# shamim-hussain/egt

Hardware: AMD Instinct MI355X
Metric: graphs/sec EGT fwd+bwd, ZINC-500K padded N=64 (higher is better)
Workload: dtype f32; 1 GPU; zinc500k_n64: attention-block stack (h,e,mask)->(h',e') x Ly, fwd+bwd + param grads; scope=stack, graphs_per_gpu=128, global_batch=128, N=64, Dh=64, De=64, H=8, d=8, Ly=10, parallelism=dp1, grad_allreduce_bytes=740480, backend=none (single process), flat_grad_adopted=True, flat_grad_bound=True, collective_in_graph=False

## Files before the change

egt_amd/_lib.py:

```python
from __future__ import annotations

import ctypes as C
import os

_HERE = os.path.dirname(os.path.abspath(__file__))
LIB_PATH = os.environ.get("EGT_AMD_LIB") or os.path.join(_HERE, "lib", "libegt_amd.so")

ABI_VERSION = 4
EGT_OK = 0
EGT_E_NULL, EGT_E_SHAPE, EGT_E_DTYPE, EGT_E_FLAGS, EGT_E_HIP, EGT_E_WORKSPACE, EGT_E_RCCL = -1, -2, -3, -4, -5, -6, -7
EGT_F32 = 0
EGT_BF16 = 1
F_EDGE_INPUT, F_GATE_INPUT, F_ATTN_MASK, F_SCALE_DEGREE = 0x001, 0x002, 0x004, 0x008
F_SCALER_LINEAR, F_TRAINING, F_CLIP = 0x010, 0x020, 0x040
ATTN_WS_SHARED = 0x1
EP_LAYERNORM, EP_GATES = 0x1, 0x2
ACT_NONE, ACT_LRELU, ACT_RELU, ACT_ELU = 0, 1, 2, 3
BF_GATE, BF_ATTN_MASK, BF_TRAINING, BF_CLIP, BF_NO_EDGE_LN, BF_SEED_DEVICE = 0x1, 0x2, 0x4, 0x8, 0x10, 0x20
BF_STATIC_EDGE = 0x40


class AttnDesc(C.Structure):
    _fields_ = [("B", C.c_int32), ("N", C.c_int32), ("H", C.c_int32), ("d", C.c_int32),
                ("dtype", C.c_int32), ("flags", C.c_uint32),
# ... 151 lines not shown
    "egt_dp_init": (C.c_int, [_VP, C.c_int32, C.c_int32]),
    "egt_dp_allreduce": (C.c_int, [_VP, C.c_size_t, C.c_int32, _VP]),
    "egt_dp_world": (C.c_int, []),
    "egt_dp_rank": (C.c_int, []),
    "egt_dp_finalize": (C.c_int, []),
    "egt_prof_enable": (C.c_int, [C.c_int]),
    "egt_prof_filter": (C.c_int, [C.c_char_p]),
    "egt_prof_stride": (C.c_int, [C.c_int]),
    "egt_prof_read": (C.c_int, [C.c_char_p, C.POINTER(C.c_int64), C.POINTER(C.c_double)]),
    "egt_prof_names": (C.c_int, [C.c_char_p, C.c_size_t]),
    "egt_prof_collect_graph": (C.c_int, [C.c_int]),
    "egt_prof_forget_graphs": (C.c_int, []),
    "egt_block_supported": (C.c_int, [C.POINTER(BlockDesc)]),
    "egt_block_bwd_kernel": (C.c_char_p, [C.POINTER(BlockDesc)]),
    "egt_block_launch_form": (C.c_char_p, [C.POINTER(BlockDesc)]),
    "egt_block_saved_bytes": (C.c_size_t, [C.POINTER(BlockDesc)]),
    "egt_block_workspace_bytes": (C.c_size_t, [C.POINTER(BlockDesc)]),
    "egt_block_fwd": (C.c_int, [C.POINTER(BlockDesc), C.POINTER(BlockParams)] + [_VP] * 10),
    "egt_block_bwd": (C.c_int, [C.POINTER(BlockDesc), C.POINTER(BlockParams)] + [_VP] * 10
                      + [C.POINTER(BlockParams)] + [_VP] * 2),
    "egt_stack_saved_bytes": (C.c_size_t, [C.POINTER(BlockDesc), C.c_int32]),
    "egt_stack_workspace_bytes": (C.c_size_t, [C.POINTER(BlockDesc), C.c_int32]),
    "egt_stack_fwd": (C.c_int, [C.POINTER(BlockDesc), C.c_int32, C.POINTER(BlockParams)] + [_VP] * 9),
    "egt_stack_bwd": (C.c_int, [C.POINTER(BlockDesc), C.c_int32, C.POINTER(BlockParams)] + [_VP] * 9
                      + [C.POINTER(BlockParams)] + [_VP] * 2),
    "egt_pair_supported": (C.c_int, [C.POINTER(BlockDesc)]),
    "egt_pair_workspace_bytes": (C.c_size_t, [C.POINTER(BlockDesc)]),
    "egt_pair_fwd": (C.c_int, [C.POINTER(BlockDesc), C.POINTER(BlockParams)] + [_VP] * 8),
    "egt_pair_bwd": (C.c_int, [C.POINTER(BlockDesc), C.POINTER(BlockParams)] + [_VP] * 9
                     + [C.POINTER(BlockParams)] + [_VP] * 2),
# ... 45 lines not shown
```

egt_amd/csrc/egt_block.h:

```cpp
#pragma once
#include "egt_common.h"

typedef float v4f __attribute__((ext_vector_type(4)));
#define MFMA(a, b, c) __builtin_amdgcn_mfma_f32_16x16x4f32((a), (b), (c), 0, 0, 0)

#define BH 8
#define QKVP 192

struct BlockArgs {
  int B, N, De, DK, Dh;
  uint32_t flags;
  int bf16;
  float clip_lo, clip_hi, scale, ln_eps;
  uint32_t rm_thr, s0, s1;
  const uint32_t* sd;
  int rng_rm;
  int TL, NLR;
  int NQP;
  int epi;
  int RGF;
  int xcd;
  int pro;
  const float *up_h, *up_nm_g, *up_Wqkv, *up_dh_out, *up_dqp, *up_dkvp;
  float *up_dqkv_sv, *up_spart;
  float *sbo;
  int spart_n, sbo_n;
  int wpart_n;
  int guard;
  unsigned* dbg; unsigned dbg_t0;
  int prep;
  const float *nx_nm_g, *nx_nm_b, *nx_Wqkv, *nx_bqkv;
  float* wfrag;
  const float *up_wfrag, *nx_wfrag;
  float* nx_qkvp;
  const float *ne_g, *ne_b, *Wg, *bg, *We, *be, *nm_g, *nm_b, *Wqkv, *bqkv, *Wo, *bo, *Wr, *br;
  const float *h, *e, *M;
  const uint8_t *km, *rm;
  float *h_out, *e_out;
  float *v_att, *stats, *qkvp;
  float *pw;
  float *dvp, *dqp, *dkvp, *epart, *ered;
  float *spart, *wpart;
  float *dqkv_sv;
  const float *dh_out, *de_out;
// ... 6 lines not shown
template <int DE>
struct Geo {
  static constexpr int TILES = (DE + 15) / 16;
  static constexpr int DEP = TILES * 16;
  static constexpr int NSLOT = DE / 4;
  static constexpr int TILE_FLOATS = 16 * DE;
  static constexpr int NF4 = 4 * DE;
  static constexpr int EP = DEP * 16 + 16 + DEP * 16;
};

__host__ __device__ inline int col_is_gate(int i) { return ((i & 1) == 0); }
__host__ __device__ inline int col_head(int i) { return 2 * (i >> 2) + ((i >> 1) & 1); }


#define BWD_TL 16
int egt_device_cus();
#define NODE_RC 32
#define WFRAG_BWQ 0
#define WFRAG_BWO 12288
#define WFRAG_FWO 16384
#define WFRAG_FWQ 20480
#define WFRAG_FLOATS 32768

size_t egt_narrow_fwd_lds(int nw);
size_t egt_narrow_bwd_lds(int nw);
void egt_narrow_launch_fwd(BlockArgs& a, int nw, bool half, const EgtLaunch& s, hipStream_t st);
void egt_narrow_launch_bwd(BlockArgs& a, int nw, const EgtLaunch& s, hipStream_t st);


void egt_node_launch_pre(BlockArgs& a, hipStream_t st);
// ... 8 lines not shown
```

egt_amd/csrc/egt_block.hip:

```cpp
#include "egt_common.h"

#include <stdio.h>
#include <stdlib.h>
#include <string.h>
#include <vector>

#include "egt_block.h"
#include "egt_tile.h"

#include "egt_block_dev.h"
#include "egt_dma.h"

#include "egt_block_fwd.h"
#include "egt_block_bwd.h"



struct EgtBlockEnv {
  bool no_narrow_fwd, no_narrow_bwd;
  int bwd_mm;
  int bwd_tl, fwd_rows;
  int nrw_fwd_waves, nrw_bwd_waves, nrw_fwd_half;
};
static bool env_flag_raw(const char* name) {
  const char* v = getenv(name);
  return v && v[0] && v[0] != '0';
}
static int env_int(const char* name, int unset) {
  const char* v = getenv(name);
  return v ? atoi(v) : unset;
}
static const EgtBlockEnv& block_env() {
  static const EgtBlockEnv e = [] {
    EgtBlockEnv v{};
    v.no_narrow_fwd = env_flag_raw("EGT_NO_NARROW_FWD") || env_flag_raw("EGT_NO_NARROW");
    v.no_narrow_bwd = env_flag_raw("EGT_NO_NARROW_BWD") || env_flag_raw("EGT_NO_NARROW");
    const char* mm = getenv("EGT_BWD_MATMUL");
    v.bwd_mm = (mm && !strcmp(mm, "bf16x3")) ? EGT_MM_BF16X3 : EGT_MM_F32;
    v.bwd_tl = env_int("EGT_BWD_TL", 0);
    v.fwd_rows = env_int("EGT_FWD_ROWS", 0);
    v.nrw_fwd_waves = env_int("EGT_NRW_FWD_WAVES", 0);
    v.nrw_bwd_waves = env_int("EGT_NRW_BWD_WAVES", 0);
    v.nrw_fwd_half = env_int("EGT_NRW_FWD_HALF", -1);
    return v;
  }();
  return e;
}
int egt_device_cus() {
  static const int n = [] {
    int dev = 0, cu = 256;
    if (hipGetDevice(&dev) == hipSuccess) (void)hipDeviceGetAttribute(&cu, hipDeviceAttributeMultiprocessorCount, dev);
    return cu > 0 ? cu : 256;
  }();
  return n;
}

static int block_check(const egt_block_desc* d, bool report) {
#define BAD(code, ...) do { if (report) egt_set_error(__VA_ARGS__); return (code); } while (0)
// ... 29 lines not shown

struct BlockPlan {
  bool ml;
  bool full;
  FwdKernel fwd;
  EgtLaunch fl;
  int fwd_nw;
  bool fwd_half;
  bool kvl;
  bool epi_ok;
  int RGF;
  BwdKernel bwd;
  EgtLaunch bl;
  int bwd_nw;
  int mm;
  int TL, NLR, nwg_bwd, EP;
  size_t v_att, stats, qkvp, pw_sv, wfrag_sv, saved_total;
  size_t dvp, dqp, dkvp, dqp_sz, dkvp_sz, common_total;
  size_t pw, epart, spart, sbo, wpart, ered, dqkv, dhbuf, layer_total;
};

template <int DE>
static BlockPlan plan_for(const egt_block_desc* d, bool ml) {
  using GG = Geo<DE>;
  const EgtBlockEnv& E = block_env();
  const int B = d->B, N = d->N, cus = egt_device_cus();
  const int groups = (N + BWD_TL - 1) / BWD_TL;
  BlockPlan P{};
  P.ml = ml;
  P.full = (N % 16) == 0;
// ... 29 lines not shown
  P.epi_ok = P.fwd != FwdKernel::tile || P.kvl;

  if (E.bwd_tl >= 4 && E.bwd_tl <= BWD_TL) P.TL = E.bwd_tl;
  else if (DE != 8) {
    const int g = tg > groups ? tg : groups;
    P.TL = (N + g - 1) / g;
  } else if (B * groups <= cus) {
    P.TL = BWD_TL;
    if (N > 8)
      for (int tl = 8; tl < BWD_TL; ++tl)
        if (B * ((N + tl - 1) / tl) <= cus) { P.TL = tl; break; }
  } else P.TL = (N + groups - 1) / groups;
  P.NLR = (N + P.TL - 1) / P.TL;
  P.nwg_bwd = B * P.NLR;
  P.EP = GG::EP;
  if (DE == 8 && !ml && !E.no_narrow_bwd) {
    P.bwd = BwdKernel::narrow;
    P.bwd_nw = E.nrw_bwd_waves == 8 || (E.nrw_bwd_waves != 4 && P.nwg_bwd <= cus && N >= 64) ? 8 : 4;
    P.bl = {P.nwg_bwd, 64 * P.bwd_nw, egt_narrow_bwd_lds(P.bwd_nw)};
  } else if (DE <= 16 && !ml) {
    constexpr int PWR = V4R_RR * (2 * GG::TILE_FLOATS + 256 + 192);
    P.bwd = BwdKernel::v4r;
    P.bl = {P.nwg_bwd, 256,
            ((size_t)(4 * PWR > BWD_PRO_WS ? 4 * PWR : BWD_PRO_WS) + (size_t)BWD_TL * QD_LD + 3 * GG::TILES * 256 + 3 * 2048 + 4) * 4};
  } else if (DE >= 32 && !ml && d->dtype != EGT_BF16) {
    P.bwd = BwdKernel::v5;
    P.mm = E.bwd_mm;
    P.bl = {P.nwg_bwd, 256, ((size_t)V5_AREA(DE) + (size_t)BWD_TL * QD_LD + 3 * ((GG::TILES + 1) / 2) * 512 + 4) * 4};
  } else {
    constexpr int PW = 3 * GG::TILE_FLOATS + 256 + 192;
    P.bwd = BwdKernel::v4;
    P.bl = {P.nwg_bwd, 256,
            ((size_t)(4 * PW > BWD_PRO_WS ? 4 * PW : BWD_PRO_WS) + (size_t)BWD_TL * QD_LD + 3 * ((GG::TILES + 1) / 2) * 512) * 4};
  }

  const size_t rows = (size_t)B * N;
  const int Dh = d->d * d->H;
  size_t o = 0;
  P.v_att = o; o += al(rows * Dh);
  P.stats = o; o += al(rows * BH * 4);
  P.qkvp = o; o += al(rows * QKVP);
  P.pw_sv = o; o += al((size_t)GG::DEP * 16 + 16);
  P.wfrag_sv = o; o += al(Dh <= 64 ? WFRAG_FLOATS : 0);
// ... 36 lines not shown
}

static bool host_rand_mask(const egt_block_desc* d, const uint8_t* rm) {
  return rm && (d->flags & EGT_BF_TRAINING) && d->random_mask_prob > 0.0f;
}
static bool mask_tensor(const egt_block_desc* d, const uint8_t* rm) {
  return (d->flags & EGT_BF_ATTN_MASK) || host_rand_mask(d, rm);
}

static void bind_ws(const BlockPlan& P, BlockArgs& a, float* wc, float* wl, int parity = 0) {
  a.dvp = wc + P.dvp; a.dqp = wc + P.dqp + parity * P.dqp_sz; a.dkvp = wc + P.dkvp + parity * P.dkvp_sz;
  a.epart = wl + P.epart; a.spart = wl + P.spart; a.sbo = wl + P.sbo; a.wpart = wl + P.wpart;
  a.spart_n = a.sbo_n = a.B * ((a.N + NODE_RC - 1) / NODE_RC);
  a.ered = wl + P.ered; a.dqkv_sv = wl + P.dqkv;
  a.TL = P.TL; a.NLR = P.NLR; a.NQP = 1;
  a.xcd = 1;
}

extern "C" const char* egt_block_bwd_kernel(const egt_block_desc* d) {
  if (block_check(d, false)) return nullptr;
  return g_bwd_kernel_name[(int)plan_block(d, mask_tensor(d, nullptr)).bwd];
}

extern "C" const char* egt_block_launch_form(const egt_block_desc* d) {
  if (block_check(d, false)) return nullptr;
  const BlockPlan P = plan_block(d, mask_tensor(d, nullptr));
  static const char* const fwd_name[] = {"k_narrow_fwd", "k_block_fwd_r4", "k_block_fwd"};
  static thread_local char buf[128];
  snprintf(buf, sizeof buf, "fwd=%s/%dw%s bwd=%s/%dw/tl%d", fwd_name[(int)P.fwd], P.fwd == FwdKernel::tile ? 4 : P.fwd_nw,
           P.fwd_half ? "/half" : "", g_bwd_kernel_name[(int)P.bwd], P.bwd == BwdKernel::narrow ? P.bwd_nw : 4, P.TL);
  return buf;
}

static int check_table(const egt_block_params* t, uint32_t flags, const char* what, int layer = -1) {
  const void* const* tp = reinterpret_cast<const void* const*>(t);
  for (int i = 0; i < 14; ++i) {
// ... 64 lines not shown
}
template <int DE, bool BF>
static void launch_tile_fwd(BlockArgs& a, const BlockPlan& P, hipStream_t st) {
  if (!P.kvl) {
    if (P.ml) egt_launch_planned<k_block_fwd<DE, false, true, false, BF>>("k_block_fwd", P.fl, st, a);
    else egt_launch_planned<k_block_fwd<DE, false, false, false, BF>>("k_block_fwd", P.fl, st, a);
  } else if (P.ml) egt_launch_planned<k_block_fwd<DE, true, true, false, BF>>("k_block_fwd", P.fl, st, a);
  else if (P.full) egt_launch_planned<k_block_fwd<DE, true, false, true, BF>>("k_block_fwd", P.fl, st, a);
  else egt_launch_planned<k_block_fwd<DE, true, false, false, BF>>("k_block_fwd", P.fl, st, a);
}
template <int DE>
static void launch_v5(BlockArgs& a, const BlockPlan& P, hipStream_t st) {
  if (P.mm == EGT_MM_BF16X3) {
    if (P.full) egt_launch_planned<k_block_bwd_v5<DE, EGT_MM_BF16X3, false>>("k_block_bwd", P.bl, st, a);
    else egt_launch_planned<k_block_bwd_v5<DE, EGT_MM_BF16X3, true>>("k_block_bwd", P.bl, st, a);
  } else {
    if (P.full) egt_launch_planned<k_block_bwd_v5<DE, EGT_MM_F32, false>>("k_block_bwd", P.bl, st, a);
    else egt_launch_planned<k_block_bwd_v5<DE, EGT_MM_F32, true>>("k_block_bwd", P.bl, st, a);
  }
}
template <int DE, bool BF>
static void launch_v4(BlockArgs& a, const BlockPlan& P, hipStream_t st) {
  if (P.ml) {
    if (P.full) egt_launch_planned<k_block_bwd_v4<DE, true, BF, false>>("k_block_bwd", P.bl, st, a);
    else egt_launch_planned<k_block_bwd_v4<DE, true, BF, true>>("k_block_bwd", P.bl, st, a);
  } else {
    if (P.full) egt_launch_planned<k_block_bwd_v4<DE, false, BF, false>>("k_block_bwd", P.bl, st, a);
    else egt_launch_planned<k_block_bwd_v4<DE, false, BF, true>>("k_block_bwd", P.bl, st, a);
  }
}
// ... 264 lines not shown
```

egt_amd/csrc/egt_block_bwd.h:

```cpp
#pragma once
#ifndef EGT_NT_BWD_E
#define EGT_NT_BWD_E true
#endif
#ifndef EGT_NT_BWD_DY
#define EGT_NT_BWD_DY false
#endif
#ifndef EGT_NT_BWD_ST
#define EGT_NT_BWD_ST false
#endif

template <int DE, bool ML, bool BF, bool RAG>
__global__ void __launch_bounds__(256, 2) k_block_bwd_v4(BlockArgs a) {
  seed_from_device(a);
  using G = Geo<DE>;
  typedef typename EdgeT<BF>::type ET;
  const ET* e_in = reinterpret_cast<const ET*>(a.e);
  ET* e_o = reinterpret_cast<ET*>(a.e_out);
  const ET* dey_in = reinterpret_cast<const ET*>(a.de_out);
  ET* dex_o = reinterpret_cast<ET*>(a.de);
  (void)e_in; (void)e_o; (void)dey_in; (void)dex_o;
  extern __shared__ __attribute__((aligned(16))) float sm[];
  const int lane = threadIdx.x & 63, wave = threadIdx.x >> 6;
  const int p = lane & 15, q = lane >> 4;
  const int N = a.N, TL = a.TL;
// ... 258 lines not shown
      ep[(16 * t + 4 * q + r) * 16 + p] = accT[t][r];
      ep[G::DEP * 16 + 16 + (16 * t + 4 * q + r) * 16 + p] = accR[t][r];
    }
  if (p == 0) {
#pragma unroll
    for (int r = 0; r < 4; ++r) ep[G::DEP * 16 + 4 * q + r] = ssum[r];
  }
  __syncthreads();
  float* out = a.epart + (size_t)wg * G::EP;
  for (int i = threadIdx.x; i < G::EP; i += 256)
    out[i] = (sm[i] + sm[G::EP + i]) + (sm[2 * G::EP + i] + sm[3 * G::EP + i]);
}

#define V5_AREA(DE_) ((4 * (3 * Geo<DE_>::TILE_FLOATS + 448) > 4 * Geo<DE_>::TILE_FLOATS + BWD_PRO_WS) \
                          ? 4 * (3 * Geo<DE_>::TILE_FLOATS + 448) : 4 * Geo<DE_>::TILE_FLOATS + BWD_PRO_WS)
template <int DE, int MM, bool RAG>
__global__ void __launch_bounds__(256, 2) k_block_bwd_v5(BlockArgs a) {
  seed_from_device(a);
  constexpr bool SPLIT = MM == EGT_MM_BF16X3;
  constexpr int NS = (Geo<DE>::TILES + 1) / 2;
  (void)SPLIT; (void)NS;
  using G = Geo<DE>;
  const float* e_in = a.e;
  const float* dey_in = a.de_out;
  float* dex_o = a.de;
  extern __shared__ __attribute__((aligned(16))) float sm[];
  const int lane = threadIdx.x & 63, wave = __builtin_amdgcn_readfirstlane(threadIdx.x >> 6);
  const int p = lane & 15, q = lane >> 4;
  const int N = a.N, TL = a.TL;
  const int wg = a.xcd ? egt_xcd_remap(blockIdx.x, gridDim.x) : (int)blockIdx.x;
  const int b = wg / a.NLR, lr = wg % a.NLR;
  const int l_begin = lr * TL, l_end = min(N, l_begin + TL), nl = l_end - l_begin;
// ... 5 lines not shown
  float* et0 = sm + wave * G::TILE_FLOATS;
  float* et1 = sm + 4 * G::TILE_FLOATS + wave * PW2;
  const int estr = __builtin_amdgcn_readfirstlane((int)(et1 - et0));
  float* dt = et1 + G::TILE_FLOATS;
  float* sc1 = dt + G::TILE_FLOATS;
  float* sc2 = sc1 + 256;
  constexpr int AREA = V5_AREA(DE);
  static_assert(4 * PW == 4 * G::TILE_FLOATS + 4 * PW2 && AREA >= 4 * PW && AREA >= 4 * G::TILE_FLOATS + BWD_PRO_WS, "tile area");
  float* pro_ws = sm + 4 * G::TILE_FLOATS;
  float* qd = sm + AREA;
  float* wsA = qd + TL * QD_LD;
  float* wsB = wsA + WSLAB;
  float* wsD = wsB + WSLAB;
  volatile int* pflag = reinterpret_cast<volatile int*>(wsD + WSLAB);
  if (threadIdx.x < 4) pflag[threadIdx.x] = 0;
  const unsigned et_lds = __builtin_amdgcn_readfirstlane((unsigned)(size_t)et0);
  const unsigned off0 = dma_lane_offset<DE>(lane);
  const int ntile = RAG ? (N + 15) / 16 : N / 16;
  const bool balance = RAG && ntile >= 3 && (ntile & 3) != 0;
  const int T_ = ntile * nl;
  const int t0 = balance ? (wave * T_) >> 2 : 0, t1 = balance ? ((wave + 1) * T_) >> 2 : 0;
  const bool have = balance ? t1 > t0 : wave < ntile;
  const int mt_first = balance ? t0 / nl : wave, mt_last = balance ? (t1 - 1) / nl : ntile - 1, mt_step = balance ? 1 : 4;
  const int r0_first = balance ? t0 - mt_first * nl : 0;
  float Kf[16], Vf[16];
  int kmv = 1;
#define V5_TILE_START(MT_, ROW_)                                                                                    \
  do {                                                                                                              \
    const int m0_ = (MT_) * 16, kv_ = RAG ? min(16, N - m0_) : 16;                                                  \
    if (RAG && kv_ < 16) tile_dma_ragged<DE>(et_lds, e_in + (((size_t)b * N + l_begin + (ROW_)) * N + m0_) * DE, lane, kv_); \
// ... 333 lines not shown
    float4* ko = reinterpret_cast<float4*>(a.dkvp + (((((size_t)b * a.NLR + lr) * N + m) * 2 + 0) * 4 + q) * 16);
    float4* vo = reinterpret_cast<float4*>(a.dkvp + (((((size_t)b * a.NLR + lr) * N + m) * 2 + 1) * 4 + q) * 16);
    if (balance && r1 < nl && r0 == 0) {
      while (pflag[wave + 1] == 0) __builtin_amdgcn_s_sleep(1);
      __builtin_amdgcn_fence(__ATOMIC_ACQUIRE, "workgroup");
      if (kvalid) {
#pragma unroll
        for (int i = 0; i < 4; ++i) {
          const float4 kk = ko[i], vv = vo[i];
          dKa[4*i] += kk.x; dKa[4*i+1] += kk.y; dKa[4*i+2] += kk.z; dKa[4*i+3] += kk.w;
          dVa[4*i] += vv.x; dVa[4*i+1] += vv.y; dVa[4*i+2] += vv.z; dVa[4*i+3] += vv.w;
        }
      }
    }
    if (kvalid) {
#pragma unroll
      for (int i = 0; i < 4; ++i) {
        ko[i] = make_float4(dKa[4*i], dKa[4*i+1], dKa[4*i+2], dKa[4*i+3]);
        vo[i] = make_float4(dVa[4*i], dVa[4*i+1], dVa[4*i+2], dVa[4*i+3]);
      }
    }
    if (balance && r0 > 0) {
      __builtin_amdgcn_fence(__ATOMIC_RELEASE, "workgroup");
      asm volatile("s_waitcnt vmcnt(0)" ::: "memory");
      if (lane == 0) pflag[wave] = 1;
    }
  }
#pragma unroll
  for (int r = 0; r < 4; ++r) ssum[r] = row_sum16(ssum[r]);
  __syncthreads();
  float* ep = sm + wave * G::EP;
#pragma unroll
  for (int t = 0; t < G::TILES; ++t)
#pragma unroll
// ... 344 lines not shown
```

egt_amd/csrc/egt_block_dev.h:

```cpp
#pragma once
#include "egt_block.h"
#include "egt_tile.h"

template <int DE>
__device__ __forceinline__ v4f project(const float4 (&x)[Geo<DE>::TILES],
                                       const float (&wA)[4 * Geo<DE>::TILES], v4f acc) {
  using G = Geo<DE>;
#pragma unroll
  for (int t = 0; t < G::TILES; ++t) {
    acc = MFMA(wA[4 * t + 0], x[t].x, acc);
    acc = MFMA(wA[4 * t + 1], x[t].y, acc);
    acc = MFMA(wA[4 * t + 2], x[t].z, acc);
    acc = MFMA(wA[4 * t + 3], x[t].w, acc);
  }
  return acc;

}

struct MaskRegs { float2 mv; unsigned short rb; };

__device__ __forceinline__ void seed_from_device(BlockArgs& a) {
  if (a.sd) { a.s0 ^= a.sd[0]; a.s1 ^= a.sd[1]; }
}

// ... 253 lines not shown

template <int DE, bool D64>
__device__ __forceinline__ void bwd_prologue_load_wo_va(const BlockArgs& a, int b, int l_begin, BwdProRegs& R) {
  BWD_PRO_COMMON();
  const bool iok = D64 || 16 * wave + p < Dh;
#pragma unroll
  for (int s = 0; s < 4; ++s)
    R.wo[s] = reinterpret_cast<const float4*>(a.wfrag + WFRAG_BWO)[(wave * 4 + s) * 64 + lane];
#pragma unroll
  for (int r = 0; r < 4; ++r) R.va[r] = iok ? a.v_att[rc(4 * q + r) * Dh + 16 * wave + p] : 0.f;
}
template <int DE, bool D64>
__device__ __forceinline__ void bwd_prologue_load_main(const BlockArgs& a, int b, int l_begin, BwdProRegs& R) {
  BWD_PRO_COMMON();
    const float4 z4 = make_float4(0.f, 0.f, 0.f, 0.f);
    R.hx = (D64 || (t & 15) * 4 < Dh) ? *reinterpret_cast<const float4*>(a.up_h + rc(t >> 4) * Dh + (t & 15) * 4) : z4;
#pragma unroll
    for (int i = 0; i < 4; ++i) {
      const bool ok = D64 || p + 16 * i < Dh;
      R.dho[i] = ok ? a.up_dh_out[rc(lnrow) * Dh + p + 16 * i] : 0.f;
      R.gmm[i] = ok ? a.up_nm_g[p + 16 * i] : 0.f;
    }
    {
      const float* base[3]; size_t pstride[3]; int NPu[3];
#pragma unroll
      for (int u = 0; u < 3; ++u) {
        const int i = t + u * 256, r = i / 48, pos4 = (i % 48) * 4, sx = pos4 >> 6;
        const int rr = max(min(r, nv - 1), 0);
        NPu[u] = sx == 0 ? a.NQP : a.NLR;
        base[u] = sx == 0 ? a.up_dqp + ((size_t)b * NPu[u] * N + l_begin + rr) * 64 + pos4
                          : a.up_dkvp + (((size_t)b * NPu[u] * N + l_begin + rr) * 2 + (sx - 1)) * 64 + (pos4 & 63);
        pstride[u] = sx == 0 ? (size_t)N * 64 : (size_t)N * 128;
        R.gq[u] = z4;
      }
      const int NPm = max(a.NQP, a.NLR);
      for (int p0 = 0; p0 < NPm; p0 += EGT_PRO_UNROLL) {
        float4 w[3][EGT_PRO_UNROLL];
#pragma unroll
        for (int u = 0; u < 3; ++u)
#pragma unroll
          for (int j = 0; j < EGT_PRO_UNROLL; ++j)
            w[u][j] = *reinterpret_cast<const float4*>(base[u] + (size_t)max(min(p0 + j, NPu[u] - 1), 0) * pstride[u]);
#pragma unroll
        for (int u = 0; u < 3; ++u)
#pragma unroll
          for (int j = 0; j < EGT_PRO_UNROLL; ++j) {
            const bool in = p0 + j < NPu[u];
            R.gq[u].x += in ? w[u][j].x : 0.f; R.gq[u].y += in ? w[u][j].y : 0.f;
            R.gq[u].z += in ? w[u][j].z : 0.f; R.gq[u].w += in ? w[u][j].w : 0.f;
          }
      }
#pragma unroll
      for (int u = 0; u < 3; ++u)
        if ((t + u * 256) / 48 >= nv) R.gq[u] = z4;
    }
#pragma unroll
    for (int s = 0; s < 12; ++s)
      R.wq[s] = reinterpret_cast<const float4*>(a.up_wfrag + WFRAG_BWQ)[(wave * 12 + s) * 64 + lane];
}

template <int DE, bool D64>
__device__ __forceinline__ void bwd_prologue_compute(const BlockArgs& a, float* ws, float* qd, int b, int l_begin, int wg, BwdProRegs& R) {
  float* dqs = ws;
  float* xs = dqs + 16 * 196;
  float* dls = xs + 16 * 68;
  float* dhs = dls + 16 * 68;
  float* rs = dhs + 16 * 68;
  float* dlp = rs + 16;
  static_assert(16 * 196 + 3 * 16 * 68 + 16 + 4 * 16 * 8 <= BWD_PRO_WS, "prologue scratch");
  BWD_PRO_COMMON();
  float4 (&wo)[4] = R.wo;
  float (&va)[4] = R.va;
  if (a.pro == 2) {
// ... 160 lines not shown
```

egt_amd/csrc/egt_node.hip:

```cpp
#include <stdlib.h>

#include "egt_block.h"

#define LDP 4

__device__ __forceinline__ float sum16(float v) { return row_sum16(v); }

__device__ __forceinline__ v4f mm_xw(const float* xs, int ld, const float* W, int ldw,
                                     int K, int p, int q, bool colok, v4f acc) {
#pragma unroll 4
  for (int t = 0; t < K; t += 4) {
    const float bv = colok ? W[(size_t)(t + q) * ldw + p] : 0.f;
    acc = MFMA(xs[p * ld + t + q], bv, acc);
  }
  return acc;
}
__device__ __forceinline__ v4f mm_xwt(const float* xs, int ld, const float* W, int ldw,
                                      int K, int p, int q, bool colok, v4f acc) {
#pragma unroll 4
  for (int t = 0; t < K; t += 4) {
    const float bv = colok ? W[(size_t)p * ldw + t + q] : 0.f;
    acc = MFMA(xs[p * ld + t + q], bv, acc);
  }
  return acc;
// ... 355 lines not shown
    stg_issue_rows(sV, x.dv_v_att + row0 * Dh, Dh, nr, nrp);
  }
  if (PRE) {
    stg_issue_weight(sWq, x.wq_a, Dh * D3 / 4);
    stg_issue_rows(sX, a.h + row0 * Dh, Dh, nr, nrp);
    {
      const int row = 4 * wave + q;
#pragma unroll
      for (int i = 0; i < 4; ++i) {
        const int c = p + 16 * i;
        const bool ok = row < nr && c < Dh;
        dho[i] = a.dh_out[ok ? (row0 + row) * Dh + c : row0 * Dh];
        gmm[i] = a.nm_g[c < Dh ? c : 0];
      }
    }
    const int U = nrp * 48;
#pragma unroll
    for (int u = 0; u < 3; ++u) {
      const int i = t + u * 512, r = i / 48, pos4 = (i % 48) * 4, sx = pos4 >> 6;
      const bool ok = i < U && r < nr;
      const int rc = ok ? r : 0;
      float4 acc4 = make_float4(0.f, 0.f, 0.f, 0.f);
      const int np = sx == 0 ? a.NQP : a.NLR;
      const float* base = sx == 0 ? a.dqp + ((size_t)b * a.NQP * N + r0 + rc) * 64 + pos4
                                  : a.dkvp + (((size_t)b * a.NLR * N + r0 + rc) * 2 + (sx - 1)) * 64 + (pos4 & 63);
      const size_t pstride = sx == 0 ? (size_t)N * 64 : (size_t)N * 128;
      if (NP > 0) {
#pragma unroll
        for (int pi = 0; pi < NP; ++pi) {
          const float4 w = *reinterpret_cast<const float4*>(base + pi * pstride);
          acc4.x += w.x; acc4.y += w.y; acc4.z += w.z; acc4.w += w.w;
        }
      } else {
        const int npmax = max(a.NQP, a.NLR);
#pragma unroll 4
        for (int pi = 0; pi < npmax; ++pi) {
          const float4 w = *reinterpret_cast<const float4*>(base + min(pi, np - 1) * pstride);
          const float f = pi < np ? 1.0f : 0.0f;
          acc4.x = fmaf(w.x, f, acc4.x); acc4.y = fmaf(w.y, f, acc4.y);
          acc4.z = fmaf(w.z, f, acc4.z); acc4.w = fmaf(w.w, f, acc4.w);
        }
      }
      gq[u] = sel4(ok, acc4);
    }
  } else {
    stg_issue_rows(sX, x.dv_dh_src + row0 * Dh, Dh, nr, nrp);
  }
  if (DV) { stg_pin(sWo); stg_pin(sV); }
  stg_pin(sX);
  if (PRE) {
    stg_pin(sWq);
#pragma unroll
// ... 276 lines not shown
        for (int r = 0; r < 4; ++r) {
          const int i = kt * 16 + 4 * q + r;
          if (i < Dh && c < Dh) part[Dh * D3 + i * Dh + c] = accO[j][r];
        }
      }
    }
  }
}

struct SumSeg { const float* src; float* dst; int n, np, stride, blk0; };
#define SUM_MAX_SEG 77
struct SumArgs { SumSeg seg[SUM_MAX_SEG]; int nseg; };

#define SUM_G 8
#define SUM_U 8
__global__ void __launch_bounds__(32 * SUM_G) k_sum_segments(SumArgs s) {
  __shared__ float red[SUM_G][32];
  int lo = 0, hi = s.nseg - 1;
  while (lo < hi) {
    const int mid = (lo + hi + 1) >> 1;
    if (s.seg[mid].blk0 <= (int)blockIdx.x) lo = mid; else hi = mid - 1;
  }
  const SumSeg sg = s.seg[lo];
  const int ol = threadIdx.x & 31, pg = threadIdx.x >> 5;
  const int o = ((int)blockIdx.x - sg.blk0) * 32 + ol;
  float v[SUM_U];
#pragma unroll
  for (int k = 0; k < SUM_U; ++k) v[k] = 0.f;
  if (o < sg.n) {
    const float* __restrict__ src = sg.src + o;
    int pi = pg;
    for (; pi + SUM_G * (SUM_U - 1) < sg.np; pi += SUM_G * SUM_U) {
      float w[SUM_U];
#pragma unroll
      for (int k = 0; k < SUM_U; ++k) w[k] = src[(size_t)(pi + SUM_G * k) * sg.stride];
#pragma unroll
      for (int k = 0; k < SUM_U; ++k) v[k] += w[k];
    }
    if (pi < sg.np) {
      float w[SUM_U];
#pragma unroll
      for (int k = 0; k < SUM_U; ++k) w[k] = src[(size_t)min(pi + SUM_G * k, sg.np - 1) * sg.stride];
#pragma unroll
      for (int k = 0; k < SUM_U; ++k) v[k] += pi + SUM_G * k < sg.np ? w[k] : 0.f;
    }
  }
  red[pg][ol] = ((v[0] + v[1]) + (v[2] + v[3])) + ((v[4] + v[5]) + (v[6] + v[7]));
  __syncthreads();
  if (pg == 0 && o < sg.n) {
    float r[SUM_G];
#pragma unroll
    for (int g = 0; g < SUM_G; ++g) r[g] = red[g][ol];
#pragma unroll
    for (int w = 1; w < SUM_G; w *= 2)
#pragma unroll
      for (int g = 0; g < SUM_G; g += 2 * w) r[g] += r[g + w];
    sg.dst[o] = r[0];
  }
}

struct EdgeGradLayer {
  const float *ne_g, *ne_b, *Wg, *We, *ered;
  float *g_ne_g, *g_ne_b, *g_Wg, *g_bg, *g_We, *g_be, *g_Wr, *g_br;
};
#define EPG_MAX_LAYERS 16
#define EPG_MAX_DE 64
struct EdgeGradArgs { EdgeGradLayer L[EPG_MAX_LAYERS]; int De; uint32_t flags; };

__global__ void __launch_bounds__(256) k_edge_param_grads(EdgeGradArgs ga) {
  constexpr int EPM = 2 * EPG_MAX_DE * 16 + 16, EU = (EPM + 255) / 256, WU = (EPG_MAX_DE * BH + 255) / 256;
  __shared__ float er[EPM], wg[EPG_MAX_DE * BH], we[EPG_MAX_DE * BH], gam[EPG_MAX_DE], bet[EPG_MAX_DE];
  const EdgeGradLayer a = ga.L[blockIdx.x];
  const bool gated = (ga.flags & EGT_BF_GATE) != 0;
// ... 143 lines not shown
    PrepArgs pa{};
    pa.De = as[0].De; pa.Dh = as[0].Dh; pa.flags = as[0].flags;
    for (int l = 0; l < nl; ++l) {
      const BlockArgs& a = as[l0 + l];
      pa.L[l] = PrepLayer{a.ne_g, a.ne_b, a.Wg, a.bg, a.We, a.be, a.pw, a.Wqkv, a.Wo, a.wfrag};
    }
    EGT_LAUNCH("k_edge_prep", k_edge_prep, dim3(nl), dim3(256), 0, st, pa);
  }
}

void egt_node_launch_reduce(BlockArgs* as, int n, int nwg_bwd, int EP, hipStream_t st) {
  for (int l0 = 0; l0 < n; l0 += 11) {
    const int nl = (n - l0 < 11) ? (n - l0) : 11;
    SumArgs s{};
    int nblk = 0, k = 0;
    auto seg = [&](const float* src, float* dst, int cnt, int npart, int stride) {
      s.seg[k] = SumSeg{src, dst, cnt, npart, stride, nblk};
      nblk += (cnt + 31) / 32;
      ++k;
    };
    for (int l = l0; l < l0 + nl; ++l) {
      BlockArgs& a = as[l];
      const int Dh = a.Dh, D3 = 3 * Dh, SP = D3 + 2 * Dh;
      const int nwc = a.wpart_n, WS = Dh * D3 + Dh * Dh;
      seg(a.wpart, a.g_Wqkv, Dh * D3, nwc, WS);
      seg(a.wpart + Dh * D3, a.g_Wo, Dh * Dh, nwc, WS);
      seg(a.spart, a.g_bqkv, D3, a.spart_n, SP);
      seg(a.spart + D3, a.g_nm_g, Dh, a.spart_n, SP);
      seg(a.spart + D3 + Dh, a.g_nm_b, Dh, a.spart_n, SP);
      seg(a.sbo, a.g_bo, Dh, a.sbo_n, Dh);
      seg(a.epart, a.ered, (a.flags & EGT_BF_STATIC_EDGE) ? EP / 2 + 8 : EP, nwg_bwd, EP);
    }
    s.nseg = k;
// ... 15 lines not shown
```

include/egt_amd.h:

```cpp
#ifndef EGT_AMD_H_
#define EGT_AMD_H_

#include <stddef.h>
#include <stdint.h>

#ifdef __cplusplus
extern "C" {
#endif

#define EGT_ABI_VERSION 4

#define EGT_OK 0
#define EGT_E_NULL (-1)
#define EGT_E_SHAPE (-2)
#define EGT_E_DTYPE (-3)
#define EGT_E_FLAGS (-4)
#define EGT_E_HIP (-5)
#define EGT_E_WORKSPACE (-6)
#define EGT_E_RCCL (-7)

#define EGT_F32 0
#define EGT_BF16 1

#define EGT_F_EDGE_INPUT 0x001u
// ... 125 lines not shown
  const void* dense_edge_b_kernel;
  const void* dense_edge_b_bias;
  const void* norm_mha_gamma;
  const void* norm_mha_beta;
  const void* dense_qkv_kernel;
  const void* dense_qkv_bias;
  const void* dense_mha_kernel;
  const void* dense_mha_bias;
  const void* dense_edge_r_kernel;
  const void* dense_edge_r_bias;
} egt_block_params;

int egt_block_supported(const egt_block_desc* desc);
const char* egt_block_bwd_kernel(const egt_block_desc* desc);
const char* egt_block_launch_form(const egt_block_desc* desc);
size_t egt_block_saved_bytes(const egt_block_desc* desc);
size_t egt_block_workspace_bytes(const egt_block_desc* desc);

int egt_block_fwd(const egt_block_desc* desc, const egt_block_params* params,
                  const void* h, const void* e, const uint8_t* key_mask,
                  const void* attn_mask, const uint8_t* rand_mask, void* h_out,
                  void* e_out, void* saved, void* workspace, void* stream);

int egt_block_bwd(const egt_block_desc* desc, const egt_block_params* params,
                  const void* h, const void* e, const uint8_t* key_mask,
                  const void* attn_mask, const uint8_t* rand_mask,
                  const void* saved, const void* d_h_out, const void* d_e_out,
                  void* d_h, void* d_e, const egt_block_params* grads,
                  void* workspace, void* stream);

// ... 171 lines not shown
```

Before: 79080 graphs/s.

## Skip dV partial stores/loads for masked keys and vectorize partial-sum reduction

In the DE=64 v5 backward kernel, dV partials are no longer stored for key rows whose key mask is zero when gates are on. The downstream prologue and node backward read a packed bitmask of zero-mask rows and skip loading those dV partials. The segment-sum reduction kernel also gains a float4 path that processes four outputs per thread for aligned segments, enabled by default. This cuts global memory traffic in the backward hand-off, at the cost of extra mask decoding and more template variants. It relies on unwritten partials never being read, which is consistent only when all consumers apply the same mask.

Result: no change. 78920 graphs/s (-0.2%).

```diff
diff --git a/egt_amd/_lib.py b/egt_amd/_lib.py
--- a/egt_amd/_lib.py
+++ b/egt_amd/_lib.py
@@ -189,6 +189,7 @@
     "egt_block_supported": (C.c_int, [C.POINTER(BlockDesc)]),
     "egt_block_bwd_kernel": (C.c_char_p, [C.POINTER(BlockDesc)]),
     "egt_block_launch_form": (C.c_char_p, [C.POINTER(BlockDesc)]),
+    "egt_block_bwd_handoff": (C.c_int, [C.POINTER(BlockDesc)]),
     "egt_block_saved_bytes": (C.c_size_t, [C.POINTER(BlockDesc)]),
     "egt_block_workspace_bytes": (C.c_size_t, [C.POINTER(BlockDesc)]),
     "egt_block_fwd": (C.c_int, [C.POINTER(BlockDesc), C.POINTER(BlockParams)] + [_VP] * 10),
diff --git a/egt_amd/csrc/egt_block.h b/egt_amd/csrc/egt_block.h
--- a/egt_amd/csrc/egt_block.h
+++ b/egt_amd/csrc/egt_block.h
@@ -27,7 +27,8 @@
   int spart_n, sbo_n;
   int wpart_n;
   int guard;
-  unsigned* dbg; unsigned dbg_t0;
+  unsigned* dbg;
+  unsigned hoff;
   int prep;
   const float *nx_nm_g, *nx_nm_b, *nx_Wqkv, *nx_bqkv;
   float* wfrag;
@@ -64,6 +65,30 @@
 
 
 #define BWD_TL 16
+#define EGT_HO_DV 1u
+#define EGT_HO_SUM4 2u
+#ifdef __HIPCC__
+template <int ND>
+__device__ __forceinline__ uint32_t egt_km_zero_bits(const uint8_t* km, size_t first, int n) {
+  typedef const __attribute__((address_space(4))) uint32_t* cptr;
+  const uintptr_t a0 = reinterpret_cast<uintptr_t>(km) + first;
+  cptr w = (cptr)(a0 & ~(uintptr_t)3);
+  const int sh = (int)(a0 & 3), nd = (sh + n + 3) >> 2;
+  uint32_t bits = 0;
+#pragma unroll
+  for (int d = 0; d < ND; ++d) {
+    if (d < nd) {
+      const uint32_t v = w[d];
+#pragma unroll
+      for (int k = 0; k < 4; ++k) {
+        const int r = 4 * d + k - sh;
+        if (r >= 0 && r < n && ((v >> (8 * k)) & 0xFFu) == 0) bits |= 1u << (r & 31);
+      }
+    }
+  }
+  return bits;
+}
+#endif
 int egt_device_cus();
 #define NODE_RC 32
 #define WFRAG_BWQ 0
diff --git a/egt_amd/csrc/egt_block.hip b/egt_amd/csrc/egt_block.hip
--- a/egt_amd/csrc/egt_block.hip
+++ b/egt_amd/csrc/egt_block.hip
@@ -21,6 +21,7 @@
   int bwd_mm;
   int bwd_tl, fwd_rows;
   int nrw_fwd_waves, nrw_bwd_waves, nrw_fwd_half;
+  unsigned handoff;
 };
 static bool env_flag_raw(const char* name) {
   const char* v = getenv(name);
@@ -42,6 +43,7 @@
     v.nrw_fwd_waves = env_int("EGT_NRW_FWD_WAVES", 0);
     v.nrw_bwd_waves = env_int("EGT_NRW_BWD_WAVES", 0);
     v.nrw_fwd_half = env_int("EGT_NRW_FWD_HALF", -1);
+    v.handoff = (unsigned)env_int("EGT_BWD_HANDOFF", 3) & 3u;
     return v;
   }();
   return e;
@@ -101,6 +103,7 @@
   EgtLaunch bl;
   int bwd_nw;
   int mm;
+  unsigned hoff;
   int TL, NLR, nwg_bwd, EP;
   size_t v_att, stats, qkvp, pw_sv, wfrag_sv, saved_total;
   size_t dvp, dqp, dkvp, dqp_sz, dkvp_sz, common_total;
@@ -160,6 +163,7 @@
   P.NLR = (N + P.TL - 1) / P.TL;
   P.nwg_bwd = B * P.NLR;
   P.EP = GG::EP;
+  P.hoff = E.handoff & EGT_HO_SUM4;
   if (DE == 8 && !ml && !E.no_narrow_bwd) {
     P.bwd = BwdKernel::narrow;
     P.bwd_nw = E.nrw_bwd_waves == 8 || (E.nrw_bwd_waves != 4 && P.nwg_bwd <= cus && N >= 64) ? 8 : 4;
@@ -173,6 +177,7 @@
     P.bwd = BwdKernel::v5;
     P.mm = E.bwd_mm;
     P.bl = {P.nwg_bwd, 256, ((size_t)V5_AREA(DE) + (size_t)BWD_TL * QD_LD + 3 * ((GG::TILES + 1) / 2) * 512 + 4) * 4};
+    if (DE == 64 && P.full && (N / 16) % 4 == 0 && P.mm == EGT_MM_F32) P.hoff |= E.handoff & EGT_HO_DV;
   } else {
     constexpr int PW = 3 * GG::TILE_FLOATS + 256 + 192;
     P.bwd = BwdKernel::v4;
@@ -239,12 +244,18 @@
   a.spart_n = a.sbo_n = a.B * ((a.N + NODE_RC - 1) / NODE_RC);
   a.ered = wl + P.ered; a.dqkv_sv = wl + P.dqkv;
   a.TL = P.TL; a.NLR = P.NLR; a.NQP = 1;
+  a.hoff = P.hoff;
   a.xcd = 1;
 }
 
 extern "C" const char* egt_block_bwd_kernel(const egt_block_desc* d) {
   if (block_check(d, false)) return nullptr;
   return g_bwd_kernel_name[(int)plan_block(d, mask_tensor(d, nullptr)).bwd];
+}
+
+extern "C" int egt_block_bwd_handoff(const egt_block_desc* d) {
+  if (block_check(d, false)) return -1;
+  return (int)plan_block(d, mask_tensor(d, nullptr)).hoff;
 }
 
 extern "C" const char* egt_block_launch_form(const egt_block_desc* d) {
@@ -339,6 +350,8 @@
   if (P.mm == EGT_MM_BF16X3) {
     if (P.full) egt_launch_planned<k_block_bwd_v5<DE, EGT_MM_BF16X3, false>>("k_block_bwd", P.bl, st, a);
     else egt_launch_planned<k_block_bwd_v5<DE, EGT_MM_BF16X3, true>>("k_block_bwd", P.bl, st, a);
+  } else if (DE == 64 && (P.hoff & EGT_HO_DV)) {
+    if constexpr (DE == 64) egt_launch_planned<k_block_bwd_v5<DE, EGT_MM_F32, false, EGT_HO_DV>>("k_block_bwd", P.bl, st, a);
   } else {
     if (P.full) egt_launch_planned<k_block_bwd_v5<DE, EGT_MM_F32, false>>("k_block_bwd", P.bl, st, a);
     else egt_launch_planned<k_block_bwd_v5<DE, EGT_MM_F32, true>>("k_block_bwd", P.bl, st, a);
diff --git a/egt_amd/csrc/egt_block_bwd.h b/egt_amd/csrc/egt_block_bwd.h
--- a/egt_amd/csrc/egt_block_bwd.h
+++ b/egt_amd/csrc/egt_block_bwd.h
@@ -296,8 +296,9 @@
 
 #define V5_AREA(DE_) ((4 * (3 * Geo<DE_>::TILE_FLOATS + 448) > 4 * Geo<DE_>::TILE_FLOATS + BWD_PRO_WS) \
                           ? 4 * (3 * Geo<DE_>::TILE_FLOATS + 448) : 4 * Geo<DE_>::TILE_FLOATS + BWD_PRO_WS)
-template <int DE, int MM, bool RAG>
+template <int DE, int MM, bool RAG, unsigned HO = 0>
 __global__ void __launch_bounds__(256, 2) k_block_bwd_v5(BlockArgs a) {
+  static_assert(HO == 0 || (!RAG && MM == 0), "the lighter hand-off: whole tiles, exact fp32 products");
   seed_from_device(a);
   constexpr bool SPLIT = MM == EGT_MM_BF16X3;
   constexpr int NS = (Geo<DE>::TILES + 1) / 2;
@@ -333,6 +334,7 @@
   float* wsD = wsB + WSLAB;
   volatile int* pflag = reinterpret_cast<volatile int*>(wsD + WSLAB);
   if (threadIdx.x < 4) pflag[threadIdx.x] = 0;
+  const bool dv_skip = (HO & EGT_HO_DV) != 0 && gated;
   const unsigned et_lds = __builtin_amdgcn_readfirstlane((unsigned)(size_t)et0);
   const unsigned off0 = dma_lane_offset<DE>(lane);
   const int ntile = RAG ? (N + 15) / 16 : N / 16;
@@ -696,10 +698,11 @@
       }
     }
     if (kvalid) {
+      const bool vst = !(dv_skip && kmv == 0);
 #pragma unroll
       for (int i = 0; i < 4; ++i) {
         ko[i] = make_float4(dKa[4*i], dKa[4*i+1], dKa[4*i+2], dKa[4*i+3]);
-        vo[i] = make_float4(dVa[4*i], dVa[4*i+1], dVa[4*i+2], dVa[4*i+3]);
+        if (vst) vo[i] = make_float4(dVa[4*i], dVa[4*i+1], dVa[4*i+2], dVa[4*i+3]);
       }
     }
     if (balance && r0 > 0) {
diff --git a/egt_amd/csrc/egt_block_dev.h b/egt_amd/csrc/egt_block_dev.h
--- a/egt_amd/csrc/egt_block_dev.h
+++ b/egt_amd/csrc/egt_block_dev.h
@@ -291,6 +291,8 @@
 __device__ __forceinline__ void bwd_prologue_load_main(const BlockArgs& a, int b, int l_begin, BwdProRegs& R) {
   BWD_PRO_COMMON();
     const float4 z4 = make_float4(0.f, 0.f, 0.f, 0.f);
+    uint32_t kmz = 0;
+    if (a.km && (a.flags & EGT_BF_GATE) && (a.hoff & EGT_HO_DV)) kmz = egt_km_zero_bits<5>(a.km, row0, nv);
     R.hx = (D64 || (t & 15) * 4 < Dh) ? *reinterpret_cast<const float4*>(a.up_h + rc(t >> 4) * Dh + (t & 15) * 4) : z4;
 #pragma unroll
     for (int i = 0; i < 4; ++i) {
@@ -298,16 +300,22 @@
       R.dho[i] = ok ? a.up_dh_out[rc(lnrow) * Dh + p + 16 * i] : 0.f;
       R.gmm[i] = ok ? a.up_nm_g[p + 16 * i] : 0.f;
     }
+#pragma unroll
+    for (int s = 0; s < 12; ++s)
+      R.wq[s] = reinterpret_cast<const float4*>(a.up_wfrag + WFRAG_BWQ)[(wave * 12 + s) * 64 + lane];
     {
       const float* base[3]; size_t pstride[3]; int NPu[3];
 #pragma unroll
       for (int u = 0; u < 3; ++u) {
         const int i = t + u * 256, r = i / 48, pos4 = (i % 48) * 4, sx = pos4 >> 6;
         const int rr = max(min(r, nv - 1), 0);
-        NPu[u] = sx == 0 ? a.NQP : a.NLR;
-        base[u] = sx == 0 ? a.up_dqp + ((size_t)b * NPu[u] * N + l_begin + rr) * 64 + pos4
-                          : a.up_dkvp + (((size_t)b * NPu[u] * N + l_begin + rr) * 2 + (sx - 1)) * 64 + (pos4 & 63);
-        pstride[u] = sx == 0 ? (size_t)N * 64 : (size_t)N * 128;
+        const int np = sx == 0 ? a.NQP : a.NLR;
+        const bool none = sx == 2 && ((kmz >> rr) & 1u);
+        base[u] = sx == 0 ? a.up_dqp + ((size_t)b * np * N + l_begin + rr) * 64 + pos4
+                          : a.up_dkvp + (((size_t)b * np * N + l_begin + rr) * 2 + (sx - 1)) * 64 + (pos4 & 63);
+        if (none) base[u] = a.up_dkvp;
+        pstride[u] = none ? 0 : sx == 0 ? (size_t)N * 64 : (size_t)N * 128;
+        NPu[u] = none ? 0 : np;
         R.gq[u] = z4;
       }
       const int NPm = max(a.NQP, a.NLR);
@@ -331,9 +339,6 @@
       for (int u = 0; u < 3; ++u)
         if ((t + u * 256) / 48 >= nv) R.gq[u] = z4;
     }
-#pragma unroll
-    for (int s = 0; s < 12; ++s)
-      R.wq[s] = reinterpret_cast<const float4*>(a.up_wfrag + WFRAG_BWQ)[(wave * 12 + s) * 64 + lane];
 }
 
 template <int DE, bool D64>
diff --git a/egt_amd/csrc/egt_node.hip b/egt_amd/csrc/egt_node.hip
--- a/egt_amd/csrc/egt_node.hip
+++ b/egt_amd/csrc/egt_node.hip
@@ -393,6 +393,8 @@
         gmm[i] = a.nm_g[c < Dh ? c : 0];
       }
     }
+    uint32_t kmz = 0;
+    if (a.km && (a.flags & EGT_BF_GATE) && (a.hoff & EGT_HO_DV)) kmz = egt_km_zero_bits<9>(a.km, row0, nr);
     const int U = nrp * 48;
 #pragma unroll
     for (int u = 0; u < 3; ++u) {
@@ -400,21 +402,24 @@
       const bool ok = i < U && r < nr;
       const int rc = ok ? r : 0;
       float4 acc4 = make_float4(0.f, 0.f, 0.f, 0.f);
-      const int np = sx == 0 ? a.NQP : a.NLR;
-      const float* base = sx == 0 ? a.dqp + ((size_t)b * a.NQP * N + r0 + rc) * 64 + pos4
-                                  : a.dkvp + (((size_t)b * a.NLR * N + r0 + rc) * 2 + (sx - 1)) * 64 + (pos4 & 63);
+      const int npa = sx == 0 ? a.NQP : a.NLR;
+      const int np = (sx == 2 && ((kmz >> rc) & 1u)) ? 0 : npa;
+      const float* base = sx == 0 ? a.dqp + ((size_t)b * npa * N + r0 + rc) * 64 + pos4
+                                  : a.dkvp + (((size_t)b * npa * N + r0 + rc) * 2 + (sx - 1)) * 64 + (pos4 & 63);
       const size_t pstride = sx == 0 ? (size_t)N * 64 : (size_t)N * 128;
-      if (NP > 0) {
-#pragma unroll
-        for (int pi = 0; pi < NP; ++pi) {
-          const float4 w = *reinterpret_cast<const float4*>(base + pi * pstride);
-          acc4.x += w.x; acc4.y += w.y; acc4.z += w.z; acc4.w += w.w;
-        }
+      if constexpr (NP > 0) {
+        float4 w[NP];
+#pragma unroll
+        for (int pi = 0; pi < NP; ++pi)
+          w[pi] = pi < np ? *reinterpret_cast<const float4*>(base + pi * pstride) : make_float4(0.f, 0.f, 0.f, 0.f);
+#pragma unroll
+        for (int pi = 0; pi < NP; ++pi) { acc4.x += w[pi].x; acc4.y += w[pi].y; acc4.z += w[pi].z; acc4.w += w[pi].w; }
       } else {
         const int npmax = max(a.NQP, a.NLR);
 #pragma unroll 4
         for (int pi = 0; pi < npmax; ++pi) {
-          const float4 w = *reinterpret_cast<const float4*>(base + min(pi, np - 1) * pstride);
+          float4 w = make_float4(0.f, 0.f, 0.f, 0.f);
+          if (np > 0) w = *reinterpret_cast<const float4*>(base + min(pi, np - 1) * pstride);
           const float f = pi < np ? 1.0f : 0.0f;
           acc4.x = fmaf(w.x, f, acc4.x); acc4.y = fmaf(w.y, f, acc4.y);
           acc4.z = fmaf(w.z, f, acc4.z); acc4.w = fmaf(w.w, f, acc4.w);
@@ -721,8 +726,44 @@
 
 #define SUM_G 8
 #define SUM_U 8
+__device__ __forceinline__ float sum_add(float a, float b) { return a + b; }
+__device__ __forceinline__ float4 sum_add(float4 a, float4 b) { return make_float4(a.x + b.x, a.y + b.y, a.z + b.z, a.w + b.w); }
+template <typename T>
+__device__ __forceinline__ T sum_group(const float* __restrict__ src, int pg, int np, int stride) {
+  T v[SUM_U];
+#pragma unroll
+  for (int k = 0; k < SUM_U; ++k) v[k] = T{};
+  int pi = pg;
+  for (; pi + SUM_G * (SUM_U - 1) < np; pi += SUM_G * SUM_U) {
+    T w[SUM_U];
+#pragma unroll
+    for (int k = 0; k < SUM_U; ++k) w[k] = *reinterpret_cast<const T*>(src + (size_t)(pi + SUM_G * k) * stride);
+#pragma unroll
+    for (int k = 0; k < SUM_U; ++k) v[k] = sum_add(v[k], w[k]);
+  }
+  if (pi < np) {
+    T w[SUM_U];
+#pragma unroll
+    for (int k = 0; k < SUM_U; ++k) w[k] = *reinterpret_cast<const T*>(src + (size_t)min(pi + SUM_G * k, np - 1) * stride);
+#pragma unroll
+    for (int k = 0; k < SUM_U; ++k) v[k] = sum_add(v[k], pi + SUM_G * k < np ? w[k] : T{});
+  }
+  return sum_add(sum_add(sum_add(v[0], v[1]), sum_add(v[2], v[3])), sum_add(sum_add(v[4], v[5]), sum_add(v[6], v[7])));
+}
+template <typename T>
+__device__ __forceinline__ T sum_across(const T (*red)[32], int ol) {
+  T r[SUM_G];
+#pragma unroll
+  for (int g = 0; g < SUM_G; ++g) r[g] = red[g][ol];
+#pragma unroll
+  for (int w = 1; w < SUM_G; w *= 2)
+#pragma unroll
+    for (int g = 0; g < SUM_G; g += 2 * w) r[g] = sum_add(r[g], r[g + w]);
+  return r[0];
+}
 __global__ void __launch_bounds__(32 * SUM_G) k_sum_segments(SumArgs s) {
-  __shared__ float red[SUM_G][32];
+  __shared__ float4 red4[SUM_G][32];
+  float (*red)[32] = reinterpret_cast<float (*)[32]>(&red4[0][0]);
   int lo = 0, hi = s.nseg - 1;
   while (lo < hi) {
     const int mid = (lo + hi + 1) >> 1;
@@ -730,40 +771,20 @@
   }
   const SumSeg sg = s.seg[lo];
   const int ol = threadIdx.x & 31, pg = threadIdx.x >> 5;
+  if (sg.n < 0) {
+    const int n = -sg.n, o = ((int)blockIdx.x - sg.blk0) * 128 + 4 * ol;
+    red4[pg][ol] = o < n ? sum_group<float4>(sg.src + o, pg, sg.np, sg.stride) : make_float4(0.f, 0.f, 0.f, 0.f);
+    __syncthreads();
+    if (pg == 0 && o < n) {
+      const float4 r = sum_across<float4>(red4, ol);
+      sg.dst[o] = r.x; sg.dst[o + 1] = r.y; sg.dst[o + 2] = r.z; sg.dst[o + 3] = r.w;
+    }
+    return;
+  }
   const int o = ((int)blockIdx.x - sg.blk0) * 32 + ol;
-  float v[SUM_U];
-#pragma unroll
-  for (int k = 0; k < SUM_U; ++k) v[k] = 0.f;
-  if (o < sg.n) {
-    const float* __restrict__ src = sg.src + o;
-    int pi = pg;
-    for (; pi + SUM_G * (SUM_U - 1) < sg.np; pi += SUM_G * SUM_U) {
-      float w[SUM_U];
-#pragma unroll
-      for (int k = 0; k < SUM_U; ++k) w[k] = src[(size_t)(pi + SUM_G * k) * sg.stride];
-#pragma unroll
-      for (int k = 0; k < SUM_U; ++k) v[k] += w[k];
-    }
-    if (pi < sg.np) {
-      float w[SUM_U];
-#pragma unroll
-      for (int k = 0; k < SUM_U; ++k) w[k] = src[(size_t)min(pi + SUM_G * k, sg.np - 1) * sg.stride];
-#pragma unroll
-      for (int k = 0; k < SUM_U; ++k) v[k] += pi + SUM_G * k < sg.np ? w[k] : 0.f;
-    }
-  }
-  red[pg][ol] = ((v[0] + v[1]) + (v[2] + v[3])) + ((v[4] + v[5]) + (v[6] + v[7]));
+  red[pg][ol] = o < sg.n ? sum_group<float>(sg.src + o, pg, sg.np, sg.stride) : 0.f;
   __syncthreads();
-  if (pg == 0 && o < sg.n) {
-    float r[SUM_G];
-#pragma unroll
-    for (int g = 0; g < SUM_G; ++g) r[g] = red[g][ol];
-#pragma unroll
-    for (int w = 1; w < SUM_G; w *= 2)
-#pragma unroll
-      for (int g = 0; g < SUM_G; g += 2 * w) r[g] += r[g + w];
-    sg.dst[o] = r[0];
-  }
+  if (pg == 0 && o < sg.n) sg.dst[o] = sum_across<float>(red, ol);
 }
 
 struct EdgeGradLayer {
@@ -937,9 +958,11 @@
     const int nl = (n - l0 < 11) ? (n - l0) : 11;
     SumArgs s{};
     int nblk = 0, k = 0;
+    const bool sum4 = (as[0].hoff & EGT_HO_SUM4) != 0;
     auto seg = [&](const float* src, float* dst, int cnt, int npart, int stride) {
-      s.seg[k] = SumSeg{src, dst, cnt, npart, stride, nblk};
-      nblk += (cnt + 31) / 32;
+      const bool v4 = sum4 && cnt % 4 == 0 && stride % 4 == 0 && (reinterpret_cast<uintptr_t>(src) & 15) == 0;
+      s.seg[k] = SumSeg{src, dst, v4 ? -cnt : cnt, npart, stride, nblk};
+      nblk += v4 ? (cnt + 127) / 128 : (cnt + 31) / 32;
       ++k;
     };
     for (int l = l0; l < l0 + nl; ++l) {
diff --git a/include/egt_amd.h b/include/egt_amd.h
--- a/include/egt_amd.h
+++ b/include/egt_amd.h
@@ -163,6 +163,7 @@
 int egt_block_supported(const egt_block_desc* desc);
 const char* egt_block_bwd_kernel(const egt_block_desc* desc);
 const char* egt_block_launch_form(const egt_block_desc* desc);
+int egt_block_bwd_handoff(const egt_block_desc* desc);
 size_t egt_block_saved_bytes(const egt_block_desc* desc);
 size_t egt_block_workspace_bytes(const egt_block_desc* desc);
 
```
